# crismolav/ggnn

Hardware: AMD Instinct MI355X
Metric: instances/sec (graphs/s) GGNN fwd+bwd, hidden=256 v=128 e=4 T=5 (higher is better)
Workload: dtype fp32; 1 GPU; configs[2]: b=256 graphs/GPU, v=128, hidden=256, e=4 (C=8), T=5, fwd+bwd; global_batch=256, parallelism=dp1

## Files before the change

ggnn_amd/csrc/ggnn_api.hip:

```cpp
#include <hip/hip_runtime.h>
#include <stdint.h>
#include <string.h>

#include <algorithm>
#include <cmath>
#include <string>
#include <vector>

#include "../../include/ggnn.h"
#include "ggnn_common.h"
#include "k_gru.h"
#include "k_gru2.h"
#include "k_fused.h"
#include "k_prep.h"
#include "k_prop.h"
#include "k_optim.h"
#include "k_wgrad.h"
#include "k_head.h"
#include "k_decode.h"
#include "k_tree.h"
#include "k_proj.h"
#include "k_marg.h"
#include "k_lapl.h"
#include "k_gemm.h"
// ... 301 lines not shown
}
bool state_bits(const Cfg& c) { return c.sd && fused_fwd(c); }
WsL ws_layout(const Cfg& c, bool training) {
  WsL L;
  memset(&L, 0, sizeof(L));
  size_t o = 0;
  const size_t N = c.N, H = c.H, T = c.T, C = c.C;
  L.nh4 = al(N * H * 4);
  L.nha = al(N * H * c.act);
  const size_t nh2 = al(N * H * 2);
  L.nhw = nh2;
  if (!c.split) {
    L.hb[0] = o; o += nh2;
    L.hb[1] = o; o += nh2;
  }
  L.Xa = o; o += L.nh4;
  if (!training) {
    L.hf[0] = o; o += L.nh4;
    L.hf[1] = o; o += L.nh4;
  } else {
    L.hfT = o; o += L.nh4 * (T + 1);
    L.hT = o;  o += L.nhw * T;
    L.XT = o;  o += L.nhw * T;
    L.rhT = o; o += L.nhw * T;
    L.r = o;   o += L.nh4 * T;
    L.u = o;   o += L.nh4 * T;
    L.c = o;   o += L.nh4 * T;
    L.dA = o;  o += L.nh4;
    L.dB = o;  o += L.nh4;
    L.dXT = o; o += L.nha;
    L.dzcT = o; o += L.nhw * T;
    L.dzgT = o; o += 2 * L.nhw * T;
    L.dMT = o;  o += C * L.nhw * T;
    L.dbp = o; o += al(T * (size_t)c.b * C * H * 4);
    L.gmax = o; o += al(GMAX_BYTES);
    if (H >= 128) {
      const WgPlan w = wg_plan(c);
      L.wpart = o; o += al((size_t)w.wgs * w.TS * w.TS * 4);
    }
    L.gbp = o; o += al((size_t)gru_bias_rows(c) * 3 * H * 4);
    L.sump = o; o += al((size_t)SUM_RCS * (3 * H + C * H) * 4);
    L.sbits = 0;
    if (fused_fwd(c)) { L.sbits = o; o += al((size_t)T * c.b * 512 * 8); }
  }
  L.total = o;
  return L;
}

template <typename T> T* P(void* base, size_t off) { return (T*)((char*)base + off); }
template <typename T> const T* P(const void* base, size_t off) { return (const T*)((const char*)base + off); }
struct ChanL {
  const int* p;
  int stride;
};
ChanL chan_lists(const Cfg& c, const void* adj, const AdjL& AL) {
  if (c.flags & GGNN_DENSE_CHANNELS) return ChanL{P<int>(adj, AL.chl_all), 0};
  return ChanL{P<int>(adj, AL.chl), c.C + 1};
}
int grid1d(long n, int bs = 256) {
  const long g = (n + bs - 1) / bs;
  return (int)std::min<long>(std::max<long>(g, 1), 8192);
}
void fill_async(void* p, unsigned char byte, size_t nbytes, hipStream_t s) {
  if (!nbytes) return;
  hipLaunchKernelGGL(k_fill, dim3(grid1d((long)((nbytes + 15) / 16))), dim3(256), 0, s, (unsigned char*)p, nbytes,
                     (unsigned)byte);
}
// ... 17 lines not shown
  hipLaunchKernelGGL(k_copy32, dim3(grid1d((n + 3) / 4)), dim3(256), 0, s, dst, src, n);
}

int gru_rt(const Cfg& c, int maxrt) {
  const long t = c.N / 32;
  if (maxrt >= 4 && t % 4 == 0) return 4;
  if (maxrt >= 2 && t % 2 == 0) return 2;
  return 1;
}

template <int V, int H, int PREC>
void launch_prop_fwd(const Cfg& c, int t, const void* hs, const u16* Ab, ChanL chl, const PackL& PL,
                     const void* pk, void* Xa, void* XT, hipStream_t s) {
  Prof p(K_PROP_FWD, s);
  hipLaunchKernelGGL((k_prop_fwd<V, H, PREC>), dim3(c.b), dim3(2 * H), 0, s, (const ActT<PREC>*)hs, Ab, chl.p, chl.stride,
                     P<u16>(pk, PL.wf(c.ed ? t : 0)), PL.loW, P<float>(pk, PL.beta), (ActT<PREC>*)Xa, (u16*)XT, c.C, c.N);
}
long wg256_kc(const Cfg& c) {
  const long N = c.N, tiles_eq = 6 + c.C;
  long KC = 8192;
  while (KC > 128 && ((N % KC) != 0 || tiles_eq * (N / KC) < 224)) KC /= 2;
  return KC;
}
bool wgrad_lists(const Cfg& c) {
  if (!(c.H == 256 && c.N % 128 == 0) || (c.flags & GGNN_DENSE_CHANNELS)) return false;
  const WgPlan w = wg_plan(c);
  const long per_t = c.ed ? w.cpt : w.nchunks;
  return (c.b + per_t - 1) / per_t <= WG_LIST_MAX && c.V % 32 == 0;
}

bool prop_f8(const Cfg& c) { return c.prec == PREC_SPLIT && c.H % 32 == 0; }

template <int V, int H, int PREC>
void launch_prop_bwd(const Cfg& c, int t, const void* dXT, const u16* AbT, const u16* deg, ChanL chl,
                     const PackL& PL, const void* pk, const float* dh_in, float* dh_out, void* dMT, float* dbp,
                     const uint32_t* gmax, const uint2* sbits, hipStream_t s) {
  Prof p(K_PROP_BWD, s);
  hipLaunchKernelGGL((k_prop_bwd<V, H, PREC>), dim3(c.b), dim3(2 * H), 0, s, (const ActT<PREC>*)dXT, AbT, deg, chl.p,
                     chl.stride,
                     P<u16>(pk, PL.wt(c.ed ? t : 0)), PL.loW, dh_in, dh_out, (u16*)dMT, dbp, c.C, c.N, c.sdrop, t - 1,
                     gmax, (int)!wgrad_lists(c), (V == 128 && H == 256) ? sbits : (const uint2*)nullptr);
}
template <int H, int RT, int PREC>
void launch_gru_fwd(const Cfg& c, int t, const void* Xa, const u16* hb, const float* hf, const PackL& PL,
                    const void* pk, float* hf_out, u16* hb_out, void* hT, float* r, float* u, float* cc, void* rhT,
                    hipStream_t s) {
  Prof p(K_GRU_FWD, s);
  if constexpr (Prec<PREC>::split && H == 256) {
    if (c.N % 128 == 0) {
      hipLaunchKernelGGL(k_gru_fwd2, dim3(c.N / 128), dim3(512), 0, s, (const float*)Xa, hf, P<u16>(pk, PL.Wg),
                         P<float>(pk, PL.bg), P<u16>(pk, PL.Wc), P<float>(pk, PL.bc), PL.loWg, PL.loWc, hf_out,
                         (u16*)hT, r, u, cc, (u16*)rhT, c.N, c.sdrop, t, c.vsh);
      return;
    }
  }
  hipLaunchKernelGGL((k_gru_fwd<H, RT, PREC>), dim3(c.N / (32 * RT)), dim3(2 * H), 0, s, (const ActT<PREC>*)Xa, hb,
                     hf, P<u16>(pk, PL.Wg), P<float>(pk, PL.bg), P<u16>(pk, PL.Wc), P<float>(pk, PL.bc), PL.loWg,
                     PL.loWc, hf_out, hb_out, (u16*)hT, r, u, cc, (u16*)rhT, c.N, c.sdrop, t, c.vsh);
}
template <int H, int RT, int PREC>
void launch_gru_bwd(const Cfg& c, const float* delta, const float* hf, const float* r, const float* u, const float* cc,
                    const PackL& PL, const void* pk, void* dXT, float* dh_out, void* dzcT, void* dzgT, float* dbc,
                    float* dbg, const uint32_t* gmax, float* bpart, const uint2* sbits, int* nwg, hipStream_t s) {
  Prof p(K_GRU_BWD, s);
  *nwg = (int)(c.N / (32 * RT));
  hipLaunchKernelGGL((k_gru_bwd<H, RT, PREC>), dim3(c.N / (32 * RT)), dim3(2 * H), 0, s, delta, hf, r, u, cc,
                     P<u16>(pk, PL.WcT), P<u16>(pk, PL.WgT), PL.loWc, PL.loWg, (ActT<PREC>*)dXT, dh_out,
                     (u16*)dzcT, (u16*)dzgT, dbc, dbg, c.N, gmax, bpart,
                     (H == 256 && c.V == 128) ? sbits : (const uint2*)nullptr, c.sdrop.scale);
}
long gru_bias_rows(const Cfg& c) { return (long)c.T * std::max<long>(c.N / 32, 1); }

#define DISPATCH_V(c, FN, H, PREC, ...)                 \
  do {                                                  \
    if ((c).V == 32) FN<32, H, PREC>(__VA_ARGS__);      \
    else if ((c).V == 64) FN<64, H, PREC>(__VA_ARGS__); \
    else FN<128, H, PREC>(__VA_ARGS__);                 \
  } while (0)
#define DISPATCH_VH(c, FN, PREC, ...)                                  \
  do {                                                                 \
    if ((c).H == 64) DISPATCH_V(c, FN, 64, PREC, __VA_ARGS__);         \
    else if ((c).H == 128) DISPATCH_V(c, FN, 128, PREC, __VA_ARGS__);  \
    else DISPATCH_V(c, FN, 256, PREC, __VA_ARGS__);                    \
  } while (0)
#define DISPATCH_RT(c, FN, H, PREC, ...)                                             \
  do {                                                                               \
    constexpr bool sp_ = Prec<PREC>::split;                                          \
    constexpr int mx_ = sp_ ? kSplitRT<FN##_tag>::value : kMaxRT<FN##_tag, H>::value; \
    const int rt_ = gru_rt(c, mx_);                                                  \
    if (mx_ >= 4 && rt_ == 4) FN<H, mx_ >= 4 ? 4 : 2, PREC>(__VA_ARGS__);            \
    else if (rt_ == 2) FN<H, 2, PREC>(__VA_ARGS__);                                  \
    else FN<H, 1, PREC>(__VA_ARGS__);                                                \
  } while (0)
#define DISPATCH_HRT(c, FN, PREC, ...)                                 \
  do {                                                                 \
    if ((c).H == 64) DISPATCH_RT(c, FN, 64, PREC, __VA_ARGS__);        \
    else if ((c).H == 128) DISPATCH_RT(c, FN, 128, PREC, __VA_ARGS__); \
    else DISPATCH_RT(c, FN, 256, PREC, __VA_ARGS__);                   \
  } while (0)

struct launch_gru_fwd_tag {};
struct launch_gru_bwd_tag {};
// ... 133 lines not shown
                  float* dbeta, float* dWg, float* dbg, float* dWc, float* dbc, hipStream_t s) {
  const WsL L = ws_layout(c, true);
  const PackL PL = pack_layout(c);
  const AdjL AL = adj_layout(c);
  const long N = c.N, H = c.H;
  const bool use_bias = (c.flags & GGNN_USE_EDGE_BIAS) != 0;
  if (H < 128) return fail(GGNN_EUNSUP, "weight gradients need hidden >= 128");

  const uint32_t* gmax = P<const uint32_t>(ws, L.gmax);
  {
    Prof p(K_IO, s);
    absmax(dhT, (long)c.b * c.vin * H, P<uint32_t>(ws, L.gmax), s);
  }
  float* dA = P<float>(ws, L.dA);
  float* dB = P<float>(ws, L.dB);
  const bool dense = c.vin == c.V;
  const uint2* sb = state_bits(c) ? P<const uint2>(ws, L.sbits) : nullptr;
  const bool in_place = dense && (!c.sd || sb);
  if (!in_place) {
    Prof p(K_IO, s);
    hipLaunchKernelGGL(k_pad_state, dim3(grid1d(N / 4 * H)), dim3(256), 0, s, dhT, c.vin, c.V, c.H, dA, (u16*)nullptr, N, 0,
                       c.sdrop, c.T - 1, gmax);
  }
  const long gb_stride = std::max<long>(N / 32, 1);
  int gb_nwg = 0;
  for (int t = c.T - 1; t >= 0; --t) {
    const bool first = t == c.T - 1 && in_place, last = t == 0 && dense;
    const float* delta = first ? dhT : dA;
    float* dh_out = last ? dh0 : dA;
    DISPATCH_HRT(c, launch_gru_bwd, PREC, c, delta, P<float>(ws, L.hfT + L.nh4 * t), P<float>(ws, L.r + L.nh4 * t),
                 P<float>(ws, L.u + L.nh4 * t), P<float>(ws, L.c + L.nh4 * t), PL, pack, P<void>(ws, L.dXT), dB,
                 P<void>(ws, L.dzcT + L.nhw * t), P<void>(ws, L.dzgT + 2 * L.nhw * t), dbc, dbg,
                 first ? gmax : (const uint32_t*)nullptr, P<float>(ws, L.gbp) + (size_t)t * gb_stride * 3 * H,
                 (first && c.sd) ? sb + (size_t)t * c.b * 512 : (const uint2*)nullptr, &gb_nwg, s);
    DISPATCH_VH(c, launch_prop_bwd, PREC, c, t, P<void>(ws, L.dXT), P<u16>(adj, AL.AbT), P<u16>(adj, AL.deg),
                chan_lists(c, adj, AL), PL, pack,
                dB, dh_out, P<void>(ws, L.dMT + (size_t)c.C * L.nhw * t),
                use_bias ? P<float>(ws, L.dbp) + (size_t)t * c.b * c.C * c.H : nullptr,
                last ? gmax : (const uint32_t*)nullptr, sb, s);
  }
  if (int e = wgrad_impl<PREC>(c, adj, ws, 0, c.T, dW, dWg, dWc, s)) return e;
  {
    Prof p(K_IO, s);
    if (!dense)
      hipLaunchKernelGGL(k_unpad_state, dim3(grid1d((long)c.b * c.vin * H)), dim3(256), 0, s, dA, c.vin, c.V, c.H, dh0,
                         (long)c.b, gmax);
    SumPlan sp(P<float>(ws, L.sump));
    sp.rows(P<const float>(ws, L.gbp), c.T, gb_nwg, gb_stride, 3 * H, dbg, dbc, 2 * H).ugmax = gmax;
    if (use_bias)
      sp.rows(P<const float>(ws, L.dbp), 1, c.T * c.b, c.T * c.b, (long)c.C * H, dbeta, dbeta, (long)c.C * H).ugmax = gmax;
    if (int e = sp.launch(s)) return e;
  }

  LAUNCHCHK();
  return GGNN_OK;
}

template <int PREC>
int wgrad_impl(const Cfg& c, const void* adj, void* ws, int t0, int nt, float* dW, float* dWg, float* dWc,
               hipStream_t s) {
  const WsL L = ws_layout(c, true);
  const long N = c.N, H = c.H;
  if (H < 128) return fail(GGNN_EUNSUP, "weight gradients need hidden >= 128");
  if (t0 != 0 || nt != c.T) return fail(GGNN_EINVAL, "weight gradients: stored over all timesteps at once");
  WgArgs a;
  memset(&a, 0, sizeof(a));
  int np = 0, tiles = 0;
  const long sa = (long)(L.nhw / 2);
  const bool big = H == 256 && N % 128 == 0;
  const int TS = big ? 256 : 128;
  const WgPlan wp = wg_plan(c);
  int wgs = 0;
  auto add = [&](size_t Poff, long stepP, size_t Qoff, long stepQ, float* out, int ldO, int M, int Nn, int nb = 1,
                 long sQb = 0, long sOb = 0) {
    WgProb& p = a.p[np++];
    p.P = P<u16>(ws, Poff) + (long)t0 * stepP;
    p.Q = P<u16>(ws, Qoff) + (long)t0 * stepQ;
    p.out = out;
    p.ldP = N; p.ldQ = N; p.stepP = stepP; p.stepQ = stepQ; p.sQb = sQb; p.sOb = sOb;
    p.ldO = ldO; p.M = M; p.N = Nn; p.tiles_n = Nn / TS; p.tiles_b = (M / TS) * p.tiles_n;
    p.sPb = 0; p.pdiv = 1; p.T = nt;
    p.tile_begin = tiles;
    tiles += nb * p.tiles_b;
// ... 979 lines not shown
```

ggnn_amd/csrc/k_gru.h:

```cpp
#pragma once
#include "ggnn_common.h"

constexpr int kGbAux = kNT;

constexpr int GF_UNROLL = 2, GB_UNROLL = 2;
constexpr int GB_DEPTH = 2;

constexpr int GB_GROUP = 4;

template <int H, int RT, int PREC>
__global__ void __launch_bounds__(2 * H)
k_gru_fwd(const ActT<PREC>* __restrict__ Xa, const u16* __restrict__ hb16, const float* __restrict__ hf,
          const u16* __restrict__ Wgp, const float* __restrict__ bg, const u16* __restrict__ Wcp,
          const float* __restrict__ bc, long wlo_g, long wlo_c, float* __restrict__ hf_out, u16* __restrict__ hb_out,
          u16* __restrict__ hT_out, float* __restrict__ r_out, float* __restrict__ u_out,
          float* __restrict__ c_out, u16* __restrict__ rhT_out, long N, Drop dr, int t, int vsh) {
  dr = drop_resolve(dr);
  constexpr bool SPLIT = Prec<PREC>::split, F16 = Prec<PREC>::f16;
  constexpr int NS = H / 32, NT = 64 * NS, KS = H / 16, R = 32 * RT, HCH = H / 8, KSG = 2 * KS;
  typedef Swz<HCH> SH;
  constexpr int NIMG = SPLIT ? 2 : 1;
  constexpr int IMG = R * H * 2;
  __shared__ __attribute__((aligned(16))) char smem[2 * NIMG * IMG];
  char* x_hi = smem;
// ... 138 lines not shown
        st_col4w<PREC>(rhT_out + wg_off(n, row0 + rt * 32 + 4 * hh, H) + 8 * q, au[rt][4 * q], au[rt][4 * q + 1],
                       au[rt][4 * q + 2], au[rt][4 * q + 3]);
    }
    if (hT_out) {
#pragma unroll
      for (int q = 0; q < 4; ++q)
        st_col4w<PREC>(hT_out + wg_off(n, row0 + rt * 32 + 4 * hh, H) + 8 * q, ac[rt][4 * q], ac[rt][4 * q + 1],
                       ac[rt][4 * q + 2], ac[rt][4 * q + 3]);
    }
  }
  if constexpr (!SPLIT) {
    __syncthreads();
    for (int q = tid; q < R * HCH; q += NT) {
      const int row = q / HCH, ch = q % HCH;
      st16(hb_out + (row0 + row) * H + ch * 8, ld16(h_hi + SH::off(row, ch)));
    }
  }
  TSMARK(0, 5);
}

template <int PREC>
DEV void gb_mma(f32x16& a1, f32x16& a2, frag ah, frag al, const F2& w) {
  mma_xb<PREC>(a1, ah, al, w.a);
  mma_xb<PREC>(a2, ah, al, w.b);
}

template <int H, int RT, int PREC>
__global__ void __launch_bounds__(2 * H, RT == 1 ? 2 : 1)
k_gru_bwd(const float* __restrict__ delta, const float* __restrict__ hf, const float* __restrict__ rin,
          const float* __restrict__ uin, const float* __restrict__ cin, const u16* __restrict__ WcTp,
          const u16* __restrict__ WgTp, long wlo_c, long wlo_g, ActT<PREC>* __restrict__ dXT,
          float* __restrict__ dh_out, u16* __restrict__ dzcT, u16* __restrict__ dzgT,
          float* __restrict__ dbc, float* __restrict__ dbg, long N, const uint32_t* __restrict__ gmax,
          float* __restrict__ bpart, const uint2* __restrict__ sbits, float sscale) {
  constexpr bool SPLIT = Prec<PREC>::split, F16 = Prec<PREC>::f16;
  constexpr int NS = H / 32, KS = H / 16, R = 32 * RT, ZCH = 2 * H / 8;
  constexpr int GBD = GB_DEPTH;
  const float ds = gscale(gmax);
  TSCLK(1, 0);
  typedef Swz<ZCH> SZ;
  typedef Swz<2 * H / 16> SZ8;
  constexpr int IMG = R * 2 * H * 2;
  __shared__ __attribute__((aligned(16))) char smem[SPLIT ? IMG + IMG / 2 : IMG];
  char* z_hi = smem;
  char* z8 = smem + IMG;
  auto zput = [&](int row, int e, float v) { *(u16*)(z_hi + SZ::eoff(row, e)) = to_limb<F16>(v); };
  auto z8_fill = [&](int c0, int nch) {
    for (int q = (int)threadIdx.x; q < R * nch; q += 2 * H) {
      const int row = q / nch, c = c0 + q % nch;
      const uint4 u[2] = {ld16(z_hi + SZ::off(row, 2 * c)), ld16(z_hi + SZ::off(row, 2 * c + 1))};
      uint32_t o[4];
#pragma unroll
      for (int i = 0; i < 4; ++i) {
        const uint4 x = u[i >> 1];
        const uint32_t w0 = (i & 1) ? x.z : x.x, w1 = (i & 1) ? x.w : x.y;
        const _Float16 h0 = __builtin_bit_cast(_Float16, (u16)(w0 & 0xffff)), h1 = __builtin_bit_cast(_Float16, (u16)(w0 >> 16));
        const _Float16 h2 = __builtin_bit_cast(_Float16, (u16)(w1 & 0xffff)), h3 = __builtin_bit_cast(_Float16, (u16)(w1 >> 16));
        o[i] = pk4_bf8((float)h0, (float)h1, (float)h2, (float)h3);
      }
      st16(z8 + SZ8::off(row, c), make_uint4(o[0], o[1], o[2], o[3]));
    }
  };

  const int tid = threadIdx.x, lane = tid & 63, ns = tid >> 6, l32 = lane & 31, hh = lane >> 5;
  const int n = ns * 32 + l32;
  const long row0 = (long)blockIdx.x * R;
  const uint32_t tbytes = R * H * 4;
// ... 141 lines not shown
        a2[rt][r] = du[rt][r] + drh * rr;
        zr[i] = drh * h * rr * (1.0f - rr);
        rsum += zr[i];
        zput(ro + 4 * hh, n, zr[i]);
      }
      st_col4w<PREC>(dzgT + twg + rt * 32 * H + 8 * q, zr[0], zr[1], zr[2], zr[3]);
    }
  }
  rsum += __shfl_xor(rsum, 32);
  if (hh == 0) {
    if (bpart) bpart[(long)blockIdx.x * 3 * H + n] = rsum;
    else atomicAdd(dbg + n, rsum);
  }
  __syncthreads();
  if constexpr (SPLIT) {
    z8_fill(0, H / 16);
    __syncthreads();
  }
  TSMARK(1, 3);

  if constexpr (SPLIT) {
    gb_f8_product(std::integral_constant<int, H / 8>{}, WgTp, (const char*)(WgTp + wlo_g));
  } else {
    auto ld2 = [&](int ks) { return F2{frag_ld(WgTp, ns, ks, 2 * KS, lane), frag_ld(WgTp, NS + ns, ks, 2 * KS, lane)}; };
    b_pipeline<2 * KS, GBD, GB_UNROLL>(ld2, [&](int ks, const auto& w) {
#pragma unroll
      for (int rt = 0; rt < RT; ++rt) {
        const frag ah = lds_frag(z_hi, SZ::off(rt * 32 + l32, 2 * ks + hh));
        gb_mma<PREC>(a1[rt], a2[rt], ah, ah, w);
      }
    });
  }
  TSMARK(1, 4);
#pragma unroll
  for (int rt = 0; rt < RT; ++rt) {
#pragma unroll
    for (int q = 0; q < 4; ++q)
      st_col4<PREC>(dXT + twg + rt * 32 * H + 8 * q, a1[rt][4 * q], a1[rt][4 * q + 1], a1[rt][4 * q + 2],
                     a1[rt][4 * q + 3]);
#pragma unroll
    for (int r = 0; r < 16; ++r) bst(pdo, a2[rt][r], vo, (rt * 32 + acc_row0(r)) * H * 4);
  }
  TSMARK(1, 5);
  TSCLK(1, 1);
}
```

ggnn_amd/csrc/k_prop.h:

```cpp
#pragma once
#include "ggnn_common.h"

constexpr int kPropAAux = kNT, kPbAux = kNT;

template <int V, int H, int PREC>
__global__ void __launch_bounds__(2 * H)
k_prop_fwd(const ActT<PREC>* __restrict__ hs_in, const u16* __restrict__ Ab, const int* __restrict__ chl, int chs,
           const u16* __restrict__ Wp, long wlo,
           const float* __restrict__ beta, ActT<PREC>* __restrict__ Xo, u16* __restrict__ XT, int C, long N) {
  constexpr bool SPLIT = Prec<PREC>::split, F16 = Prec<PREC>::f16;
  using Act = ActT<PREC>;
  constexpr int NS = H / 32, NT = 64 * NS, VT = V / 32, KS = H / 16;
  constexpr int HCH = H / 8, ACH = V / 8;
  typedef Swz<ACH> SA;
  constexpr int NIMG = SPLIT ? 2 : 1;
  constexpr int IMG = V * H * 2;
  constexpr int A_BYTES = V * V * 2;
  constexpr int NAB = (!SPLIT && NIMG * IMG + 2 * A_BYTES <= 163840) ? 2 : 1;
  __shared__ __attribute__((aligned(16))) char smem[NIMG * IMG + NAB * A_BYTES];
  char* h_hi = smem;
  char* h_lo = smem + (SPLIT ? IMG : 0);
  auto abuf_of = [&](int i) { return smem + NIMG * IMG + (NAB == 2 ? (i & 1) * A_BYTES : 0); };

  const int g = blockIdx.x, tid = threadIdx.x, lane = tid & 63, ns = tid >> 6;
// ... 58 lines not shown
  }

  if (XT) {
#pragma unroll
    for (int it = 0; it < VT; ++it)
#pragma unroll
      for (int q = 0; q < 4; ++q)
        st_col4w<PREC>(XT + wg_off(n, rowg + it * 32 + 4 * hh, H) + 8 * q, accx[it][4 * q], accx[it][4 * q + 1],
                       accx[it][4 * q + 2], accx[it][4 * q + 3]);
  }
  if constexpr (SPLIT) {
    float* xs = (float*)smem;
#pragma unroll
    for (int it = 0; it < VT; ++it)
#pragma unroll
      for (int r = 0; r < 16; ++r) xs[(it * 32 + acc_row(r, hh)) * H + n] = accx[it][r];
    __syncthreads();
    for (int q = tid; q < V * H / 4; q += NT) *(float4*)(Xo + rowg * H + q * 4) = ((const float4*)xs)[q];
  } else {
#pragma unroll
    for (int it = 0; it < VT; ++it)
#pragma unroll
      for (int r = 0; r < 16; ++r) *(u16*)(h_hi + kimg<V>(it * 32 + acc_row(r, hh), n >> 3) + (n & 7) * 2) = to_limb<F16>(accx[it][r]);
    __syncthreads();
    for (int q = tid; q < V * HCH; q += NT) {
      const int row = q / HCH, ch = q % HCH;
      st16(Xo + (rowg + row) * H + ch * 8, ld16(h_hi + kimg<V>(row, ch)));
    }
  }
}

template <int V, int H, int PREC>
__global__ void __launch_bounds__(2 * H)
k_prop_bwd(const ActT<PREC>* __restrict__ dXT, const u16* __restrict__ AbT, const u16* __restrict__ deg,
           const int* __restrict__ chl, int chs, const u16* __restrict__ WTp, long wlo, const float* __restrict__ dh_in, float* __restrict__ dh_out,
           u16* __restrict__ dMT, float* __restrict__ dbp, int C, long N, Drop dr, int tm,
           const uint32_t* __restrict__ gmax, int zdm, const uint2* __restrict__ sbits) {
  dr = drop_resolve(dr);
  TSCLK(3, 0);
  constexpr bool SPLIT = Prec<PREC>::split, F16 = Prec<PREC>::f16;
  using Act = ActT<PREC>;
  constexpr int NS = H / 32, NT = 64 * NS, VT = V / 32, KV = V / 16, KS = H / 16;
  constexpr int HCH = H / 8, ACH = V / 8;
  typedef Swz<HCH> SH;
  typedef Swz<ACH> SA;
  constexpr int NIMG = SPLIT ? 2 : 1;
  constexpr int IMG = V * H * 2, A_BYTES = V * V * 2;
  __shared__ __attribute__((aligned(16))) char smem[A_BYTES + NIMG * IMG];
  char* abuf = smem;
  char* m_hi = smem + A_BYTES;
  char* m_lo = m_hi + (SPLIT ? IMG : 0);

  const int g = blockIdx.x, tid = threadIdx.x, lane = tid & 63, ns = tid >> 6, l32 = lane & 31, hh = lane >> 5;
  const int n = ns * 32 + l32;
  const long rowg = (long)g * V;

  frag dxh[KV], dxl[KV];
#pragma unroll
  for (int s = 0; s < KV; ++s) {
    const Act* p = dXT + wg_off(n, rowg + 16 * s + 8 * hh, H);
    if constexpr (SPLIT) {
      typedef float f4v __attribute__((ext_vector_type(4)));
      const f4v a = *(const f4v*)p, b = *(const f4v*)(p + 4);
      const float x[8] = {a.x, a.y, a.z, a.w, b.x, b.y, b.z, b.w};
      dxh[s] = pk8<true>(x);
      dxl[s] = pk8_lo<true>(x);
    } else {
      dxh[s] = ld16(p);
      dxl[s] = dxh[s];
    }
  }

  const int* cl = chl + (long)g * chs;
  const int nc = cl[0];
  auto chan = [&](int i) { return cl[1 + i]; };
  const u16* ag = AbT + (long)g * C * V * V;
  if (nc > 0) glds_tile<ACH, V, NT, kPropAAux>(abuf, ag + (long)chan(0) * V * V, tid);
  const rsrc_t rdh = mkrsrc(dh_in + rowg * H, V * H * 4);
  const int vo = (4 * hh * H + n) * 4;
  const bool drop = dr.thr != 0 && tm >= 0;
  uint2 kb = make_uint2(0u, 0u);
  if (drop && sbits) kb = sbits[((long)tm * gridDim.x + g) * NT + tid];
  f32x16 adh[VT];
#pragma unroll
  for (int jt = 0; jt < VT; ++jt)
#pragma unroll
    for (int r = 0; r < 16; ++r) adh[jt][r] = bld_p<kPbAux>(rdh, vo, (jt * 32 + acc_row0(r)) * H * 4);
  __syncthreads();

  for (int ci = 0; ci < nc; ++ci) {
    const int c = chan(ci);
    v2u32 dq[VT][4];
#pragma unroll
    for (int jt = 0; jt < VT; ++jt) {
      f32x16 am = splat(0.f);
#pragma unroll
      for (int s = 0; s < KV; ++s) {
        const frag b = lds_frag(abuf, SA::off(jt * 32 + l32, 2 * s + hh));
        mma_xb<PREC>(am, dxh[s], dxl[s], b);
      }
      const int j = jt * 32 + l32;
#pragma unroll
      for (int q = 0; q < 4; ++q) {
        const int n0 = ns * 32 + 8 * q + 4 * hh;
        const uint32_t p0 = pk<F16>(am[4 * q], am[4 * q + 1]), p1 = pk<F16>(am[4 * q + 2], am[4 * q + 3]);
        const int mo = kimg<V>(j, n0 >> 3) + (n0 & 7) * 2;
        *(uint2*)(m_hi + mo) = make_uint2(p0, p1);
        if constexpr (SPLIT) {
          const int o = 8 * q + 4 * hh;
          float lo[4];
#pragma unroll
          for (int i = 0; i < 4; ++i) lo[i] = lo_part<true>(am[4 * q + i]) * (float)(1 << F8_M);
          const int m8 = kimg<V>(j, 4 * ns + (o >> 4)) + (o & 15);
          *(uint32_t*)(m_lo + m8) = pk4_bf8(am[4 * q], am[4 * q + 1], am[4 * q + 2], am[4 * q + 3]);
          *(uint32_t*)(m_lo + m8 + 2 * V * 16) = pk4_bf8(lo[0], lo[1], lo[2], lo[3]);
        }
        dq[jt][q] = quad_transpose4(p0, p1, l32 & 3);
      }
    }
    if (dbp) {
      const uint4* dg = (const uint4*)(deg + ((long)g * C + c) * V);
      f32x16 db = splat(0.f);
#pragma unroll
      for (int ss = 0; ss < KV; ++ss) {
        const uint4 d0 = dg[2 * ss], d1 = dg[2 * ss + 1];
        mma_xb<PREC>(db, dxh[ss], dxl[ss], hh ? d1 : d0);
      }
      float v = 0.f;
#pragma unroll
      for (int r = 0; r < 16; ++r) v = (r == (l32 & 15)) ? db[r] : v;
      if (l32 < 16) dbp[((long)g * C + c) * H + ns * 32 + acc_row(l32, hh)] = v;
    }
    __syncthreads();
    if (ci + 1 < nc) glds_tile<ACH, V, NT, kPropAAux>(abuf, ag + (long)chan(ci + 1) * V * V, tid);
    const u16* wt = WTp + (size_t)c * H * H;
    if constexpr (SPLIT) {
      const char* w8 = (const char*)(wt + wlo);
      auto ld_h = [&](int kb) { return F2{frag_ld(wt, ns, 2 * kb, KS, lane), frag_ld(wt, ns, 2 * kb + 1, KS, lane)}; };
      auto ld_f = [&](int kb) {
        const uint4* f = (const uint4*)(w8 + ((size_t)(ns * (KS / 2) + kb) * 64 + lane) * 32);
        return F2{f[0], f[1]};
      };
      F2 rh = ld_h(0), rf = ld_f(0);
#pragma unroll 1
      for (int kb = 0; kb < KS / 2; ++kb) {
        const int kn = min(kb + 1, KS / 2 - 1);
#pragma unroll
        for (int jt = 0; jt < VT; ++jt) {
          const int row = jt * 32 + l32;
          adh[jt] = mfma<true>(lds_frag(m_hi, kimg<V>(row, 4 * kb + hh)), rh.a, adh[jt]);
          adh[jt] = mfma<true>(lds_frag(m_hi, kimg<V>(row, 4 * kb + 2 + hh)), rh.b, adh[jt]);
        }
        rh = ld_h(kn);
        __builtin_amdgcn_sched_barrier(0);
#pragma unroll
        for (int jt = 0; jt < VT; ++jt) {
          const int row = jt * 32 + l32;
          const uint4 p0 = ld16(m_lo + kimg<V>(row, 4 * kb + 2 * hh)), p1 = ld16(m_lo + kimg<V>(row, 4 * kb + 2 * hh + 1));
          adh[jt] = mfma_f8corr(p0, p1, rf.a, rf.b, adh[jt]);
        }
        rf = ld_f(kn);
        __builtin_amdgcn_sched_barrier(0);
      }
    } else {
      auto ldb = [&](int ks) { return F2{frag_ld(wt, ns, ks, KS, lane), frag{}}; };
      auto pb = [&](int ks, const F2& w) {
#pragma unroll
        for (int jt = 0; jt < VT; ++jt) {
          const frag ah = lds_frag(m_hi, kimg<V>(jt * 32 + l32, 2 * ks + hh));
          mma<PREC>(adh[jt], ah, ah, w.a, w.b);
        }
      };
      b_pipeline<KS, 2, 1>(ldb, pb);
    }
    if (dMT) {
      const bool odd = (l32 >> 2) & 1;
      u16* dmt = dMT + (long)c * H * N;
#pragma unroll
      for (int jt = 0; jt < VT; ++jt)
#pragma unroll
        for (int qp = 0; qp < 4; qp += 2) {
          const v2u32 mine = odd ? dq[jt][qp + 1] : dq[jt][qp];
          const v2u32 send = odd ? dq[jt][qp] : dq[jt][qp + 1];
          const uint32_t r0 = (uint32_t)__builtin_amdgcn_ds_swizzle((int)send.x, 0x101F);
          const uint32_t r1 = (uint32_t)__builtin_amdgcn_ds_swizzle((int)send.y, 0x101F);
          typedef unsigned int u32x4v __attribute__((ext_vector_type(4)));
          const u32x4v out = odd ? u32x4v{r0, r1, mine.x, mine.y} : u32x4v{mine.x, mine.y, r0, r1};
          const int nn = ns * 32 + 8 * (qp + (odd ? 1 : 0)) + 4 * hh + (l32 & 3);
          __builtin_nontemporal_store(out, (u32x4v*)(dmt + wg_off(nn, rowg + jt * 32 + 8 * (l32 >> 3), H)));
        }
    }
    __syncthreads();
  }
  const rsrc_t rdo = mkrsrc(dh_out + rowg * H, V * H * 4);
  const float osc = gunscale(gmax);
#pragma unroll
  for (int jt = 0; jt < VT; ++jt) {
    uint4 dw = make_uint4(0, 0, 0, 0);
#pragma unroll
    for (int r = 0; r < 16; ++r) {
      float x = adh[jt][r] * osc;
      if (drop) {
        if (sbits) {
          const uint32_t w = (VT == 4) ? ((jt >> 1) ? kb.y : kb.x) : kb.x;
          x = ((w >> ((jt & 1) * 16 + r)) & 1u) ? x * dr.scale : 0.0f;
        } else {
          if ((r & 3) == 0) dw = state_words(dr, g, jt * 32 + acc_row0(r) + 4 * hh, n, tm);
          x = drop_apply(dr, u4_get(dw, r & 3), x);
        }
      }
      bst(rdo, x, vo, (jt * 32 + acc_row0(r)) * H * 4);
    }
  }
  if (nc < C) {
    for (int c = 0, p = 0; c < C; ++c) {
      if (p < nc && cl[1 + p] == c) {
        ++p;
        continue;
      }
      if (dMT && zdm) {
        u16* z = dMT + (long)c * H * N + rowg * H;
        for (int q = tid; q < V * H / 8; q += NT) st16(z + q * 8, make_uint4(0, 0, 0, 0));
      }
      if (dbp)
        for (int q = tid; q < H; q += NT) dbp[((long)g * C + c) * H + q] = 0.f;
    }
  }
  TSCLK(3, 1);
}
```

ggnn_amd/csrc/ggnn_common.h:

```cpp
#pragma once

#include <hip/hip_runtime.h>
#include <stdint.h>

#include <type_traits>

typedef uint16_t u16;
typedef __bf16 bf16x8 __attribute__((ext_vector_type(8)));
typedef _Float16 f16x8 __attribute__((ext_vector_type(8)));
typedef float f32x16 __attribute__((ext_vector_type(16)));
typedef uint4 frag;
typedef unsigned int v2u32 __attribute__((ext_vector_type(2)));

#define DEV __device__ __forceinline__
#define HDI __host__ __device__ inline
#ifdef GGNN_TS
__device__ unsigned long long g_ts[4][2048 * 8];
#define TSMARK(k, i) do { if (threadIdx.x == 0) g_ts[k][blockIdx.x * 8 + (i)] = __builtin_amdgcn_s_memrealtime(); } while (0)
#define TSVAL(k, i, v) do { if (threadIdx.x == 0) g_ts[k][blockIdx.x * 8 + (i)] = (unsigned long long)(v); } while (0)
__device__ unsigned long long g_clk[4][2048 * 4];
#define TSCLK(k, e) do { if (threadIdx.x == 0) { \
    g_clk[k][blockIdx.x * 4 + 2 * (e)] = __builtin_amdgcn_s_memrealtime(); \
    g_clk[k][blockIdx.x * 4 + 2 * (e) + 1] = __builtin_amdgcn_s_memtime(); } } while (0)
#else
// ... 31 lines not shown
  if constexpr (F16) return __builtin_bit_cast(uint32_t, __builtin_convertvector(v, f16x2v));
  else return __builtin_bit_cast(uint32_t, __builtin_convertvector(v, bf16x2v));
}
#ifndef GGNN_LIMB_MIX
#define GGNN_LIMB_MIX 1
#endif
template <bool F16, bool MIX = GGNN_LIMB_MIX> DEV uint32_t pk_lo(float a, float b) {
  if constexpr (F16 && MIX) {
    const uint32_t hi = pk<true>(a, b);
    uint32_t lo;
    asm("v_fma_mixlo_f16 %0, %1, 1.0, -%2 op_sel_hi:[0,0,1]" : "=v"(lo) : "v"(a), "v"(hi));
    asm("v_fma_mixhi_f16 %0, %1, 1.0, -%2 op_sel:[0,0,1] op_sel_hi:[0,0,1]\n\ts_nop 1" : "+v"(lo) : "v"(b), "v"(hi));
    return lo;
  }
  const f32x2v v = {a, b};
  f32x2v back;
  if constexpr (F16) back = __builtin_convertvector(__builtin_convertvector(v, f16x2v), f32x2v);
  else back = __builtin_convertvector(__builtin_convertvector(v, bf16x2v), f32x2v);
  const f32x2v lo = v - back;
  return pk<F16>(lo.x, lo.y);
}
template <bool F16> DEV frag pk8(const float* x) {
  return make_uint4(pk<F16>(x[0], x[1]), pk<F16>(x[2], x[3]), pk<F16>(x[4], x[5]), pk<F16>(x[6], x[7]));
}
DEV u16 lo_limb16(float v) {
  if constexpr (GGNN_LIMB_MIX) {
    const uint32_t hi = __builtin_bit_cast(u16, (_Float16)v);
    uint32_t lo;
    asm("v_fma_mixlo_f16 %0, %1, 1.0, -%2 op_sel_hi:[0,0,1]" : "=v"(lo) : "v"(v), "v"(hi));
    return (u16)lo;
  }
  return to_limb<true>(lo_part<true>(v));
}
template <bool F16, bool MIX = GGNN_LIMB_MIX> DEV frag pk8_lo(const float* x) {
  return make_uint4(pk_lo<F16, MIX>(x[0], x[1]), pk_lo<F16, MIX>(x[2], x[3]), pk_lo<F16, MIX>(x[4], x[5]),
                    pk_lo<F16, MIX>(x[6], x[7]));
}
template <bool F16> DEV float limb_elem(frag f, int j) {
  const uint32_t w = (j < 2) ? f.x : (j < 4) ? f.y : (j < 6) ? f.z : f.w;
  return from_limb<F16>((u16)((j & 1) ? (w >> 16) : (w & 0xffff)));
}

template <bool F16> DEV f32x16 mfma(frag a, frag b, f32x16 c) {
  if constexpr (F16)
    return __builtin_amdgcn_mfma_f32_32x32x16_f16(__builtin_bit_cast(f16x8, a), __builtin_bit_cast(f16x8, b), c, 0, 0, 0);
  else
    return __builtin_amdgcn_mfma_f32_32x32x16_bf16(__builtin_bit_cast(bf16x8, a), __builtin_bit_cast(bf16x8, b), c, 0, 0, 0);
}
DEV f32x16 splat(float x) {
  f32x16 r;
#pragma unroll
  for (int i = 0; i < 16; ++i) r[i] = x;
  return r;
}
DEV float sigm(float x) { return 1.0f / (1.0f + __expf(-x)); }
DEV float tanh_f(float x) { return 1.0f - 2.0f / (__expf(2.0f * x) + 1.0f); }
DEV constexpr int acc_row0(int r) { return (r & 3) + 8 * (r >> 2); }
DEV int acc_row(int r, int hh) { return acc_row0(r) + 4 * hh; }

template <bool F16> DEV frag acc_hi(const f32x16& a, int s) {
  float x[8];
#pragma unroll
  for (int j = 0; j < 8; ++j) x[j] = a[8 * s + j];
  return pk8<F16>(x);
}
template <bool F16, bool MIX = GGNN_LIMB_MIX> DEV frag acc_lo(const f32x16& a, int s) {
// ... 18 lines not shown
}
template <int PREC>
DEV void mma_xb(f32x16& acc, frag ah, frag al, frag b) {
  if constexpr (Prec<PREC>::split) acc = mfma<true>(al, b, acc);
  acc = mfma<Prec<PREC>::f16>(ah, b, acc);
}

constexpr int F8_Q = 7, F8_M = 11;
typedef int i32x8 __attribute__((ext_vector_type(8)));
DEV uint32_t pk4_bf8(float a, float b, float c, float d) {
  uint32_t w = (uint32_t)__builtin_amdgcn_cvt_pk_bf8_f32(a, b, 0, false);
  return (uint32_t)__builtin_amdgcn_cvt_pk_bf8_f32(c, d, (int)w, true);
}
DEV uint32_t pk4_fp8(float a, float b, float c, float d) {
  uint32_t w = (uint32_t)__builtin_amdgcn_cvt_pk_fp8_f32(a, b, 0, false);
  return (uint32_t)__builtin_amdgcn_cvt_pk_fp8_f32(c, d, (int)w, true);
}
DEV f32x16 mfma_f8corr(uint4 a0, uint4 a1, uint4 b0, uint4 b1, f32x16 c) {
  const i32x8 fa = {(int)a0.x, (int)a0.y, (int)a0.z, (int)a0.w, (int)a1.x, (int)a1.y, (int)a1.z, (int)a1.w};
  const i32x8 fb = {(int)b0.x, (int)b0.y, (int)b0.z, (int)b0.w, (int)b1.x, (int)b1.y, (int)b1.z, (int)b1.w};
  return __builtin_amdgcn_mfma_scale_f32_32x32x64_f8f6f4(fa, fb, c, 1, 0, 0, 127, 0, 127 - F8_Q - F8_M);
}

template <int NCH>
struct Swz {
  static constexpr int M = (NCH % 16 == 0) ? 15 : (NCH % 8 == 0) ? 7 : (NCH % 4 == 0) ? 3 : 0;
  static DEV int off(int row, int ch) { return row * NCH * 16 + ((ch ^ (row & M)) << 4); }
  static DEV int eoff(int row, int e) { return off(row, e >> 3) + ((e & 7) << 1); }
};

DEV uint4 ld16(const void* p) { return *(const uint4*)p; }
DEV void st16(void* p, uint4 v) { *(uint4*)p = v; }
DEV frag lds_frag(const char* img, int off) { return ld16(img + off); }

template <int NCH, int R, int NT, int AUX = 0>
DEV void glds_tile(char* lds, const u16* src, int tid) {
  typedef Swz<NCH> S;
  constexpr int TOT = R * NCH;
  const int lane = tid & 63;
#pragma unroll
  for (int p = 0; p < (TOT + NT - 1) / NT; ++p) {
    const int qb = p * NT + (tid & ~63);
    if (qb < TOT) {
      const int q = qb + lane, row = q / NCH, pc = q % NCH;
      __builtin_amdgcn_global_load_lds((const void*)(src + (row * NCH + (pc ^ (row & S::M))) * 8),
                                       (__attribute__((address_space(3))) void*)(lds + qb * 16), 16, 0, AUX);
    }
  }
}

DEV void glds16_asm(const void* gsrc, const char* lds_dst) {
  unsigned keep;
  const unsigned dst = __builtin_amdgcn_readfirstlane((unsigned)(uintptr_t)lds_dst);
  asm volatile("s_mov_b32 %0, m0\n\ts_mov_b32 m0, %2\n\ts_nop 0\n\tglobal_load_lds_dwordx4 %1, off\n\ts_mov_b32 m0, %0"
               : "=&s"(keep)
               : "v"(gsrc), "s"(dst)
               : "memory");
}

DEV frag frag_ld(const u16* base, int strip, int ks, int nks, int lane) {
  return ld16(base + ((size_t)(strip * nks + ks) * 64 + lane) * 8);
}

struct F2 { frag a, b; };
struct F4 { frag a, b, c, d; };
template <int KS, int D, int UNROLL = 0, typename LD, typename BODY>
// ... 174 lines not shown
```

Measured before the change: 105,700 graphs/s.

## Move per-channel bias-gradient reduction from prop_bwd into gru_bwd epilogue

Computes the beta bias gradient (deg-weighted sum of dX over nodes per channel) inside the GRU backward kernel epilogue, using the in-register a1 accumulators and MFMA against degree fragments. The per-graph partial buffer is replaced by per-workgroup partials that share the gru bias row stride. Removes the dbp reduction and its zeroing for absent channels from the prop backward kernel, shortening its inner loop. In exchange gru_bwd loads deg for every channel, which adds register pressure and work in that kernel.

Measured after the change: 105,500 graphs/s. Within noise of the previous version (-0.1%).

```diff
diff --git a/ggnn_amd/csrc/ggnn_api.hip b/ggnn_amd/csrc/ggnn_api.hip
--- a/ggnn_amd/csrc/ggnn_api.hip
+++ b/ggnn_amd/csrc/ggnn_api.hip
@@ -357,7 +357,7 @@
     L.dzcT = o; o += L.nhw * T;
     L.dzgT = o; o += 2 * L.nhw * T;
     L.dMT = o;  o += C * L.nhw * T;
-    L.dbp = o; o += al(T * (size_t)c.b * C * H * 4);
+    L.dbp = o; o += al((size_t)gru_bias_rows(c) * C * H * 4);
     L.gmax = o; o += al(GMAX_BYTES);
     if (H >= 128) {
       const WgPlan w = wg_plan(c);
@@ -441,13 +441,13 @@
 bool prop_f8(const Cfg& c) { return c.prec == PREC_SPLIT && c.H % 32 == 0; }
 
 template <int V, int H, int PREC>
-void launch_prop_bwd(const Cfg& c, int t, const void* dXT, const u16* AbT, const u16* deg, ChanL chl,
-                     const PackL& PL, const void* pk, const float* dh_in, float* dh_out, void* dMT, float* dbp,
+void launch_prop_bwd(const Cfg& c, int t, const void* dXT, const u16* AbT, ChanL chl,
+                     const PackL& PL, const void* pk, const float* dh_in, float* dh_out, void* dMT,
                      const uint32_t* gmax, const uint2* sbits, hipStream_t s) {
   Prof p(K_PROP_BWD, s);
-  hipLaunchKernelGGL((k_prop_bwd<V, H, PREC>), dim3(c.b), dim3(2 * H), 0, s, (const ActT<PREC>*)dXT, AbT, deg, chl.p,
+  hipLaunchKernelGGL((k_prop_bwd<V, H, PREC>), dim3(c.b), dim3(2 * H), 0, s, (const ActT<PREC>*)dXT, AbT, chl.p,
                      chl.stride,
-                     P<u16>(pk, PL.wt(c.ed ? t : 0)), PL.loW, dh_in, dh_out, (u16*)dMT, dbp, c.C, c.N, c.sdrop, t - 1,
+                     P<u16>(pk, PL.wt(c.ed ? t : 0)), PL.loW, dh_in, dh_out, (u16*)dMT, c.C, c.N, c.sdrop, t - 1,
                      gmax, (int)!wgrad_lists(c), (V == 128 && H == 256) ? sbits : (const uint2*)nullptr);
 }
 template <int H, int RT, int PREC>
@@ -470,13 +470,14 @@
 template <int H, int RT, int PREC>
 void launch_gru_bwd(const Cfg& c, const float* delta, const float* hf, const float* r, const float* u, const float* cc,
                     const PackL& PL, const void* pk, void* dXT, float* dh_out, void* dzcT, void* dzgT, float* dbc,
-                    float* dbg, const uint32_t* gmax, float* bpart, const uint2* sbits, int* nwg, hipStream_t s) {
+                    float* dbg, const uint32_t* gmax, float* bpart, const uint2* sbits, const u16* deg, float* dbpart,
+                    int* nwg, hipStream_t s) {
   Prof p(K_GRU_BWD, s);
   *nwg = (int)(c.N / (32 * RT));
   hipLaunchKernelGGL((k_gru_bwd<H, RT, PREC>), dim3(c.N / (32 * RT)), dim3(2 * H), 0, s, delta, hf, r, u, cc,
                      P<u16>(pk, PL.WcT), P<u16>(pk, PL.WgT), PL.loWc, PL.loWg, (ActT<PREC>*)dXT, dh_out,
                      (u16*)dzcT, (u16*)dzgT, dbc, dbg, c.N, gmax, bpart,
-                     (H == 256 && c.V == 128) ? sbits : (const uint2*)nullptr, c.sdrop.scale);
+                     (H == 256 && c.V == 128) ? sbits : (const uint2*)nullptr, c.sdrop.scale, deg, dbpart, c.C, c.vsh);
 }
 long gru_bias_rows(const Cfg& c) { return (long)c.T * std::max<long>(c.N / 32, 1); }
 
@@ -676,11 +677,11 @@
                  P<float>(ws, L.u + L.nh4 * t), P<float>(ws, L.c + L.nh4 * t), PL, pack, P<void>(ws, L.dXT), dB,
                  P<void>(ws, L.dzcT + L.nhw * t), P<void>(ws, L.dzgT + 2 * L.nhw * t), dbc, dbg,
                  first ? gmax : (const uint32_t*)nullptr, P<float>(ws, L.gbp) + (size_t)t * gb_stride * 3 * H,
-                 (first && c.sd) ? sb + (size_t)t * c.b * 512 : (const uint2*)nullptr, &gb_nwg, s);
-    DISPATCH_VH(c, launch_prop_bwd, PREC, c, t, P<void>(ws, L.dXT), P<u16>(adj, AL.AbT), P<u16>(adj, AL.deg),
+                 (first && c.sd) ? sb + (size_t)t * c.b * 512 : (const uint2*)nullptr, P<u16>(adj, AL.deg),
+                 use_bias ? P<float>(ws, L.dbp) + (size_t)t * gb_stride * c.C * H : (float*)nullptr, &gb_nwg, s);
+    DISPATCH_VH(c, launch_prop_bwd, PREC, c, t, P<void>(ws, L.dXT), P<u16>(adj, AL.AbT),
                 chan_lists(c, adj, AL), PL, pack,
                 dB, dh_out, P<void>(ws, L.dMT + (size_t)c.C * L.nhw * t),
-                use_bias ? P<float>(ws, L.dbp) + (size_t)t * c.b * c.C * c.H : nullptr,
                 last ? gmax : (const uint32_t*)nullptr, sb, s);
   }
   if (int e = wgrad_impl<PREC>(c, adj, ws, 0, c.T, dW, dWg, dWc, s)) return e;
@@ -692,7 +693,7 @@
     SumPlan sp(P<float>(ws, L.sump));
     sp.rows(P<const float>(ws, L.gbp), c.T, gb_nwg, gb_stride, 3 * H, dbg, dbc, 2 * H).ugmax = gmax;
     if (use_bias)
-      sp.rows(P<const float>(ws, L.dbp), 1, c.T * c.b, c.T * c.b, (long)c.C * H, dbeta, dbeta, (long)c.C * H).ugmax = gmax;
+      sp.rows(P<const float>(ws, L.dbp), c.T, gb_nwg, gb_stride, (long)c.C * H, dbeta, dbeta, (long)c.C * H).ugmax = gmax;
     if (int e = sp.launch(s)) return e;
   }
 
diff --git a/ggnn_amd/csrc/k_gru.h b/ggnn_amd/csrc/k_gru.h
--- a/ggnn_amd/csrc/k_gru.h
+++ b/ggnn_amd/csrc/k_gru.h
@@ -194,7 +194,8 @@
           const u16* __restrict__ WgTp, long wlo_c, long wlo_g, ActT<PREC>* __restrict__ dXT,
           float* __restrict__ dh_out, u16* __restrict__ dzcT, u16* __restrict__ dzgT,
           float* __restrict__ dbc, float* __restrict__ dbg, long N, const uint32_t* __restrict__ gmax,
-          float* __restrict__ bpart, const uint2* __restrict__ sbits, float sscale) {
+          float* __restrict__ bpart, const uint2* __restrict__ sbits, float sscale,
+          const u16* __restrict__ deg, float* __restrict__ dbpart, int C, int vsh) {
   constexpr bool SPLIT = Prec<PREC>::split, F16 = Prec<PREC>::f16;
   constexpr int NS = H / 32, KS = H / 16, R = 32 * RT, ZCH = 2 * H / 8;
   constexpr int GBD = GB_DEPTH;
@@ -402,6 +403,29 @@
     });
   }
   TSMARK(1, 4);
+  int ln = lane;
+  if (dbpart) asm volatile("" : "+v"(ln));
+  const int el = ln & 31, eh = ln >> 5;
+  frag dga[RT][2];
+  auto ld_deg = [&](int c0) {
+    const int c = c0 + el;
+    const unsigned vd = (unsigned)(((c << vsh) + 4 * eh) * 2);
+#pragma unroll
+    for (int rt = 0; rt < RT; ++rt) {
+      const long row = row0 + rt * 32;
+      const char* dg = (const char*)(deg + (((row >> vsh) * C) << vsh) + (row & ((1L << vsh) - 1)));
+#pragma unroll
+      for (int s2 = 0; s2 < 2; ++s2) {
+        uint2 d0 = make_uint2(0u, 0u), d1 = d0;
+        if (c < C) {
+          d0 = *(const uint2*)(dg + 32 * s2 + (unsigned long)vd);
+          d1 = *(const uint2*)(dg + 32 * s2 + 16 + (unsigned long)vd);
+        }
+        dga[rt][s2] = make_uint4(d0.x, d0.y, d1.x, d1.y);
+      }
+    }
+  };
+  if (dbpart) ld_deg(0);
 #pragma unroll
   for (int rt = 0; rt < RT; ++rt) {
 #pragma unroll
@@ -411,6 +435,27 @@
 #pragma unroll
     for (int r = 0; r < 16; ++r) bst(pdo, a2[rt][r], vo, (rt * 32 + acc_row0(r)) * H * 4);
   }
+  if (dbpart) {
+    char* dbo = (char*)(dbpart + (long)blockIdx.x * C * H);
+    const unsigned vs = (unsigned)((4 * eh * H + ns * 32 + el) * 4);
+    for (int c0 = 0; c0 < C; c0 += 32) {
+      if (c0) ld_deg(c0);
+      f32x16 db = splat(0.f);
+#pragma unroll
+      for (int rt = 0; rt < RT; ++rt)
+#pragma unroll
+        for (int s2 = 0; s2 < 2; ++s2)
+          mma_xa<PREC>(db, dga[rt][s2], acc_hi<F16>(a1[rt], s2), acc_lo<F16>(a1[rt], s2));
+#pragma unroll
+      for (int q = 0; q < 4; ++q) {
+        if (c0 + 8 * q >= C) break;
+#pragma unroll
+        for (int i = 0; i < 4; ++i)
+          if (c0 + 8 * q + 4 * eh + i < C)
+            *(float*)(dbo + (long)(c0 + 8 * q + i) * H * 4 + (unsigned long)vs) = db[4 * q + i];
+      }
+    }
+  }
   TSMARK(1, 5);
   TSCLK(1, 1);
 }
diff --git a/ggnn_amd/csrc/k_prop.h b/ggnn_amd/csrc/k_prop.h
--- a/ggnn_amd/csrc/k_prop.h
+++ b/ggnn_amd/csrc/k_prop.h
@@ -114,9 +114,9 @@
 
 template <int V, int H, int PREC>
 __global__ void __launch_bounds__(2 * H)
-k_prop_bwd(const ActT<PREC>* __restrict__ dXT, const u16* __restrict__ AbT, const u16* __restrict__ deg,
+k_prop_bwd(const ActT<PREC>* __restrict__ dXT, const u16* __restrict__ AbT,
            const int* __restrict__ chl, int chs, const u16* __restrict__ WTp, long wlo, const float* __restrict__ dh_in, float* __restrict__ dh_out,
-           u16* __restrict__ dMT, float* __restrict__ dbp, int C, long N, Drop dr, int tm,
+           u16* __restrict__ dMT, int C, long N, Drop dr, int tm,
            const uint32_t* __restrict__ gmax, int zdm, const uint2* __restrict__ sbits) {
   dr = drop_resolve(dr);
   TSCLK(3, 0);
@@ -200,19 +200,6 @@
         dq[jt][q] = quad_transpose4(p0, p1, l32 & 3);
       }
     }
-    if (dbp) {
-      const uint4* dg = (const uint4*)(deg + ((long)g * C + c) * V);
-      f32x16 db = splat(0.f);
-#pragma unroll
-      for (int ss = 0; ss < KV; ++ss) {
-        const uint4 d0 = dg[2 * ss], d1 = dg[2 * ss + 1];
-        mma_xb<PREC>(db, dxh[ss], dxl[ss], hh ? d1 : d0);
-      }
-      float v = 0.f;
-#pragma unroll
-      for (int r = 0; r < 16; ++r) v = (r == (l32 & 15)) ? db[r] : v;
-      if (l32 < 16) dbp[((long)g * C + c) * H + ns * 32 + acc_row(l32, hh)] = v;
-    }
     __syncthreads();
     if (ci + 1 < nc) glds_tile<ACH, V, NT, kPropAAux>(abuf, ag + (long)chan(ci + 1) * V * V, tid);
     const u16* wt = WTp + (size_t)c * H * H;
@@ -294,18 +281,14 @@
       bst(rdo, x, vo, (jt * 32 + acc_row0(r)) * H * 4);
     }
   }
-  if (nc < C) {
+  if (nc < C && dMT && zdm) {
     for (int c = 0, p = 0; c < C; ++c) {
       if (p < nc && cl[1 + p] == c) {
         ++p;
         continue;
       }
-      if (dMT && zdm) {
-        u16* z = dMT + (long)c * H * N + rowg * H;
-        for (int q = tid; q < V * H / 8; q += NT) st16(z + q * 8, make_uint4(0, 0, 0, 0));
-      }
-      if (dbp)
-        for (int q = tid; q < H; q += NT) dbp[((long)g * C + c) * H + q] = 0.f;
+      u16* z = dMT + (long)c * H * N + rowg * H;
+      for (int q = tid; q < V * H / 8; q += NT) st16(z + q * 8, make_uint4(0, 0, 0, 0));
     }
   }
   TSCLK(3, 1);
```

## Software-pipeline prop bwd A-matmul epilogue and transpose dMT via ds_read_tr16

Applied to the files above, without the earlier changes.

Restructures the k_prop_bwd message stage so LDS A-fragment loads are double-buffered and the packing/store epilogue of the previous tile is interleaved with the MFMAs of the next. It also computes the split-precision residual with a fused mix-FMA against the packed high limb. The dMT write now reads the transposed tile back from LDS with ds_read_tr16 instead of holding dq registers and using ds_swizzle exchanges. The aim is to hide epilogue latency and cut register pressure, at the cost of extra LDS reads and tighter scheduling constraints. Timestamp markers were added but are compiled out by default.

New measurement: 107,200 graphs/s before, 109,500 graphs/s after (median of 6 runs). 2.1% higher.

```diff
diff --git a/ggnn_amd/csrc/ggnn_common.h b/ggnn_amd/csrc/ggnn_common.h
--- a/ggnn_amd/csrc/ggnn_common.h
+++ b/ggnn_amd/csrc/ggnn_common.h
@@ -87,6 +87,15 @@
   }
   return to_limb<true>(lo_part<true>(v));
 }
+template <int HALF> DEV float resid16(float x, uint32_t hpk) {
+  if constexpr (GGNN_LIMB_MIX) {
+    float lo;
+    if constexpr (HALF == 0) asm("v_fma_mix_f32 %0, %1, 1.0, -%2 op_sel_hi:[0,0,1]" : "=v"(lo) : "v"(x), "v"(hpk));
+    else asm("v_fma_mix_f32 %0, %1, 1.0, -%2 op_sel:[0,0,1] op_sel_hi:[0,0,1]" : "=v"(lo) : "v"(x), "v"(hpk));
+    return lo;
+  }
+  return x - from_limb<true>((u16)(hpk >> (16 * HALF)));
+}
 template <bool F16, bool MIX = GGNN_LIMB_MIX> DEV frag pk8_lo(const float* x) {
   return make_uint4(pk_lo<F16, MIX>(x[0], x[1]), pk_lo<F16, MIX>(x[2], x[3]), pk_lo<F16, MIX>(x[4], x[5]),
                     pk_lo<F16, MIX>(x[6], x[7]));
@@ -171,6 +180,10 @@
 DEV uint4 ld16(const void* p) { return *(const uint4*)p; }
 DEV void st16(void* p, uint4 v) { *(uint4*)p = v; }
 DEV frag lds_frag(const char* img, int off) { return ld16(img + off); }
+typedef short s16x4 __attribute__((ext_vector_type(4)));
+DEV v2u32 lds_tr16(const char* p) {
+  return __builtin_bit_cast(v2u32, __builtin_amdgcn_ds_read_tr16_b64_v4i16((__attribute__((address_space(3))) s16x4*)p));
+}
 
 template <int NCH, int R, int NT, int AUX = 0>
 DEV void glds_tile(char* lds, const u16* src, int tid) {
diff --git a/ggnn_amd/csrc/k_prop.h b/ggnn_amd/csrc/k_prop.h
--- a/ggnn_amd/csrc/k_prop.h
+++ b/ggnn_amd/csrc/k_prop.h
@@ -120,6 +120,7 @@
            const uint32_t* __restrict__ gmax, int zdm, const uint2* __restrict__ sbits) {
   dr = drop_resolve(dr);
   TSCLK(3, 0);
+  TSMARK(3, 0);
   constexpr bool SPLIT = Prec<PREC>::split, F16 = Prec<PREC>::f16;
   using Act = ActT<PREC>;
   constexpr int NS = H / 32, NT = 64 * NS, VT = V / 32, KV = V / 16, KS = H / 16;
@@ -169,37 +170,63 @@
 #pragma unroll
     for (int r = 0; r < 16; ++r) adh[jt][r] = bld_p<kPbAux>(rdh, vo, (jt * 32 + acc_row0(r)) * H * 4);
   __syncthreads();
+  TSMARK(3, 1);
 
   for (int ci = 0; ci < nc; ++ci) {
     const int c = chan(ci);
-    v2u32 dq[VT][4];
-#pragma unroll
-    for (int jt = 0; jt < VT; ++jt) {
-      f32x16 am = splat(0.f);
-#pragma unroll
-      for (int s = 0; s < KV; ++s) {
-        const frag b = lds_frag(abuf, SA::off(jt * 32 + l32, 2 * s + hh));
-        mma_xb<PREC>(am, dxh[s], dxl[s], b);
-      }
-      const int j = jt * 32 + l32;
-#pragma unroll
-      for (int q = 0; q < 4; ++q) {
-        const int n0 = ns * 32 + 8 * q + 4 * hh;
-        const uint32_t p0 = pk<F16>(am[4 * q], am[4 * q + 1]), p1 = pk<F16>(am[4 * q + 2], am[4 * q + 3]);
-        const int mo = kimg<V>(j, n0 >> 3) + (n0 & 7) * 2;
-        *(uint2*)(m_hi + mo) = make_uint2(p0, p1);
+    TSMARK(3, 2);
+    {
+      constexpr int NST = VT * KV;
+      constexpr int NM = SPLIT ? 2 : 1;
+      constexpr int NP = 16 / (KV * NM);
+      auto lda = [&](int i) { return lds_frag(abuf, SA::off((i / KV) * 32 + l32, 2 * (i % KV) + hh)); };
+      frag bq[2] = {lda(0), lda(NST > 1 ? 1 : 0)};
+      f32x16 am[2];
+      uint32_t pq[2] = {0u, 0u};
+      float lq[2] = {0.f, 0.f};
+      auto piece = [&](int jt, int t, const f32x16& x) {
+        const int q = t >> 2, k = t & 3, j = jt * 32 + l32;
+        const int o = 8 * q + 4 * hh;
+        const int m8 = kimg<V>(j, 4 * ns + (o >> 4)) + (o & 15);
+        if (k == 0) {
+          const int n0 = ns * 32 + o;
+          pq[0] = pk<F16>(x[4 * q], x[4 * q + 1]);
+          pq[1] = pk<F16>(x[4 * q + 2], x[4 * q + 3]);
+          *(uint2*)(m_hi + kimg<V>(j, n0 >> 3) + (n0 & 7) * 2) = make_uint2(pq[0], pq[1]);
+        }
         if constexpr (SPLIT) {
-          const int o = 8 * q + 4 * hh;
-          float lo[4];
-#pragma unroll
-          for (int i = 0; i < 4; ++i) lo[i] = lo_part<true>(am[4 * q + i]) * (float)(1 << F8_M);
-          const int m8 = kimg<V>(j, 4 * ns + (o >> 4)) + (o & 15);
-          *(uint32_t*)(m_lo + m8) = pk4_bf8(am[4 * q], am[4 * q + 1], am[4 * q + 2], am[4 * q + 3]);
-          *(uint32_t*)(m_lo + m8 + 2 * V * 16) = pk4_bf8(lo[0], lo[1], lo[2], lo[3]);
-        }
-        dq[jt][q] = quad_transpose4(p0, p1, l32 & 3);
-      }
-    }
+          const float sc = (float)(1 << F8_M);
+          if (k == 1) *(uint32_t*)(m_lo + m8) = pk4_bf8(x[4 * q], x[4 * q + 1], x[4 * q + 2], x[4 * q + 3]);
+          if (k == 2) {
+            lq[0] = resid16<0>(x[4 * q], pq[0]) * sc;
+            lq[1] = resid16<1>(x[4 * q + 1], pq[0]) * sc;
+          }
+          if (k == 3)
+            *(uint32_t*)(m_lo + m8 + 2 * V * 16) =
+                pk4_bf8(lq[0], lq[1], resid16<0>(x[4 * q + 2], pq[1]) * sc, resid16<1>(x[4 * q + 3], pq[1]) * sc);
+        }
+      };
+#pragma unroll
+      for (int i = 0; i < NST; ++i) {
+        const int jt = i / KV, s = i % KV;
+        f32x16& acc = am[jt & 1];
+        if (s == 0) acc = splat(0.f);
+#pragma unroll
+        for (int m = 0; m < NM; ++m) {
+          if (SPLIT && m == 0) acc = mfma<true>(dxl[s], bq[i & 1], acc);
+          else acc = mfma<F16>(dxh[s], bq[i & 1], acc);
+          if (m == NM - 1 && i + 2 < NST) bq[i & 1] = lda(i + 2);
+          if (jt > 0) {
+#pragma unroll
+            for (int t = (s * NM + m) * NP; t < (s * NM + m + 1) * NP; ++t) piece(jt - 1, t, am[(jt - 1) & 1]);
+          }
+          __builtin_amdgcn_sched_barrier(0);
+        }
+      }
+#pragma unroll
+      for (int t = 0; t < 16; ++t) piece(VT - 1, t, am[(VT - 1) & 1]);
+    }
+    TSMARK(3, 3);
     if (dbp) {
       const uint4* dg = (const uint4*)(deg + ((long)g * C + c) * V);
       f32x16 db = splat(0.f);
@@ -213,6 +240,7 @@
       for (int r = 0; r < 16; ++r) v = (r == (l32 & 15)) ? db[r] : v;
       if (l32 < 16) dbp[((long)g * C + c) * H + ns * 32 + acc_row(l32, hh)] = v;
     }
+    TSMARK(3, 4);
     __syncthreads();
     if (ci + 1 < nc) glds_tile<ACH, V, NT, kPropAAux>(abuf, ag + (long)chan(ci + 1) * V * V, tid);
     const u16* wt = WTp + (size_t)c * H * H;
@@ -255,23 +283,26 @@
       };
       b_pipeline<KS, 2, 1>(ldb, pb);
     }
+    TSMARK(3, 5);
     if (dMT) {
-      const bool odd = (l32 >> 2) & 1;
-      u16* dmt = dMT + (long)c * H * N;
+      int ln = lane;
+      asm volatile("" : "+v"(ln));
+      const int gb = (ln >> 4) & 1, i16 = ln & 15, h2 = ln >> 5;
+      const int trx = kimg<V>(16 * gb + 8 * ((i16 >> 1) & 1) + 4 * gb + (i16 >> 2), h2) + 8 * (i16 & 1);
+      const int try_ = trx ^ 64;
+      u16* dmt = dMT + (long)c * H * N + wg_off(ns * 32 + 8 * h2 + (i16 & 7), rowg + 16 * gb + 8 * (i16 >> 3), H);
 #pragma unroll
       for (int jt = 0; jt < VT; ++jt)
 #pragma unroll
-        for (int qp = 0; qp < 4; qp += 2) {
-          const v2u32 mine = odd ? dq[jt][qp + 1] : dq[jt][qp];
-          const v2u32 send = odd ? dq[jt][qp] : dq[jt][qp + 1];
-          const uint32_t r0 = (uint32_t)__builtin_amdgcn_ds_swizzle((int)send.x, 0x101F);
-          const uint32_t r1 = (uint32_t)__builtin_amdgcn_ds_swizzle((int)send.y, 0x101F);
+        for (int s = 0; s < 2; ++s) {
+          const char* src = m_hi + kimg<V>(jt * 32, 4 * ns + 2 * s);
+          const v2u32 x = lds_tr16(src + trx), y = lds_tr16(src + try_);
           typedef unsigned int u32x4v __attribute__((ext_vector_type(4)));
-          const u32x4v out = odd ? u32x4v{r0, r1, mine.x, mine.y} : u32x4v{mine.x, mine.y, r0, r1};
-          const int nn = ns * 32 + 8 * (qp + (odd ? 1 : 0)) + 4 * hh + (l32 & 3);
-          __builtin_nontemporal_store(out, (u32x4v*)(dmt + wg_off(nn, rowg + jt * 32 + 8 * (l32 >> 3), H)));
-        }
-    }
+          const u32x4v out = gb ? u32x4v{y.x, y.y, x.x, x.y} : u32x4v{x.x, x.y, y.x, y.y};
+          __builtin_nontemporal_store(out, (u32x4v*)(dmt + wg_off(16 * s, jt * 32, H)));
+        }
+    }
+    TSMARK(3, 6);
     __syncthreads();
   }
   const rsrc_t rdo = mkrsrc(dh_out + rowg * H, V * H * 4);
@@ -308,5 +339,6 @@
         for (int q = tid; q < H; q += NT) dbp[((long)g * C + c) * H + q] = 0.f;
     }
   }
+  TSMARK(3, 7);
   TSCLK(3, 1);
 }
```
